# zongh5a/MDF-Net

Measured on AMD Instinct MI355X. Metric: views/sec at DTU 1600x1200x5-view x4-scale, higher is better.
Workload: dtype f32; 1 GPU; DTU eval 1600x1184 (1600x1200 cropped as load/dtueval.py:34), 5 views, 3 cost-volume stages + x2 refine = 4 output scales, hypotheses (48,24,8), batch 1 per rank, seeded random weights (pth/dtu_29.pth is not available offline); parallelism=views sharded over 1 rank(s), no collective

## Files before the change

### mdf-net_amd/csrc/conv3d.hip

```cpp
#include <cstdlib>
#include "common.h"

namespace {

typedef float f32x4 __attribute__((ext_vector_type(4)));

enum ConvMode { kS1 = 0, kS2 = 1, kTr = 2 };

struct ConvParams {
  const float* x;
  const float* wpack;
  const float* alpha;
  const float* beta;
  const float* res;
  float* y;
  int B, Di, Hi, Wi, Do, Ho, Wo;
  int relu;
  long long m_total;
  unsigned nblk;
  int stat_mode;
  const float* stat_y;
  const float* stat_aux;
  double* stat_out;
  int stat_slices;
// ... 708 lines not shown
  const int KPL = (Cin >= 16) ? 4 : (Cin == 8 ? 2 : 1), CK = 4 * KPL, NCH = Cin / CK, KW = KHW + RW - 1;
  int r = i;
  const int s = r % KPL; r /= KPL;
  const int n = r % 16; r /= 16;
  const int qq = r % 4; r /= 4;
  const int ch = r % NCH; r /= NCH;
  const int kwp = r % KW, kdh = r / KW;
  const int phase = n / Cout, cout = n % Cout, cin = ch * CK + KPL * qq + s;
  const int kw = kwp - phase;
  return (phase < RW && cin < Cin_mem && kw >= 0 && kw < KHW) ? src.at(cout, cin, kdh * KHW + kw) : 0.f;
}

__device__ __forceinline__ int pack_wino_total(int Cin, int Cout, int nkd) { return nkd * (Cin / 16) * 16 * ((Cout + 15) / 16) * 64 * 4; }
__device__ __forceinline__ float pack_wino_elem(const WSrc& src, int i, int Cin, int Cout, int nkd) {
  const int NCH = Cin / 16, NT = (Cout + 15) / 16;
  const float G[4][3] = {{1.f, 0.f, 0.f}, {.5f, .5f, .5f}, {.5f, -.5f, .5f}, {0.f, 0.f, 1.f}};
  int r = i;
  const int s = r % 4; r /= 4;
  const int m = r % 16; r /= 16;
  const int qq = r % 4; r /= 4;
  const int nt = r % NT; r /= NT;
  const int ab = r % 16; r /= 16;
  const int ch = r % NCH; r /= NCH;
  const int kd = r;
  const int a = ab >> 2, b = ab & 3;
  const int cout = nt * 16 + m, cin = ch * 16 + 4 * qq + s;
  float v = 0.f;
  if (cout < Cout) {
    for (int y = 0; y < 3; ++y)
      for (int x = 0; x < 3; ++x) v += G[a][y] * G[b][x] * src.at(cout, cin, kd * 9 + y * 3 + x);
  }
  return v;
}

__device__ __forceinline__ float pack_wd_elem(const WSrc& src, int i, int Cin) {
  const int KPL = (Cin >= 16) ? 4 : 2, CK = 4 * KPL, NCH = Cin / CK;
  const float G[4][3] = {{1.f, 0.f, 0.f}, {.5f, .5f, .5f}, {.5f, -.5f, .5f}, {0.f, 0.f, 1.f}};
  int r = i;
  const int s = r % KPL; r /= KPL;
  const int m = r % 16; r /= 16;
  const int qq = r % 4; r /= 4;
  const int ab = r % 16; r /= 16;
  const int ch = r % NCH; r /= NCH;
  const int j = r;
  const int a = ab >> 2, b = ab & 3;
  const int cout = m & 7, kd = j - (m >> 3), cin = ch * CK + KPL * qq + s;
  float v = 0.f;
  if (kd >= 0 && kd < 3) {
    for (int y = 0; y < 3; ++y)
      for (int x = 0; x < 3; ++x) v += G[a][y] * G[b][x] * src.at(cout, cin, kd * 9 + y * 3 + x);
  }
  return v;
}

__device__ __forceinline__ int pack_tr_total(int Cin, int Cout) {
  const int KPL = (Cin >= 16) ? 4 : 2, CK = 4 * KPL, NCH = Cin / CK, NT = (2 * Cout + 15) / 16;
  return 18 * NCH * NT * 64 * KPL;
}
__device__ __forceinline__ float pack_tr_elem(const WSrc& src, int i, int Cin, int Cout) {
  const int KPL = (Cin >= 16) ? 4 : 2, CK = 4 * KPL, NCH = Cin / CK, NT = (2 * Cout + 15) / 16;
  int r = i;
  const int s = r % KPL; r /= KPL;
  const int n = r % 16; r /= 16;
  const int qq = r % 4; r /= 4;
  const int nt = r % NT; r /= NT;
  const int ch = r % NCH; r /= NCH;
  const int tap = r;
  const int kd = tap / 6, kh = (tap / 2) % 3, ow = tap & 1;
  const int row = nt * 16 + n, cin = ch * CK + KPL * qq + s;
  if (row >= 2 * Cout) return 0.f;
  const int pw = row / Cout, cout = row % Cout;
  const int kw = (pw == 0) ? (ow == 0 ? 1 : -1) : (ow == 0 ? 2 : 0);
  return kw >= 0 ? src.at(cout, cin, (kd * 3 + kh) * 3 + kw) : 0.f;
}

__host__ __device__ inline int rw_of(int Cout) { return Cout == 8 ? 2 : (Cout == 4 ? 4 : 0); }
__host__ __device__ inline bool wino_built(int Cin, int Cout) {
  return ((Cout == 16 || Cout == 32) && (Cin == 16 || Cin == 32)) || (Cin == 16 && Cout == 8);
}
__host__ __device__ inline bool wino2d_built(int Cin, int Cout) {
  return (Cin == 16 && Cout == 16) || (Cin == 32 && Cout == 32) || (Cin == 64 && Cout == 64) || (Cin == 16 && Cout == 32) || (Cin == 32 && Cout == 64);
}
__host__ __device__ inline bool wd_built(int Cin, int Cout) { return Cout == 8 && (Cin == 8 || Cin == 16); }
__host__ __device__ inline bool k5w_built(int Cin, int Cout) { return (Cin == 16 && Cout == 32) || (Cin == 8 && Cout == 16); }
__host__ __device__ inline int padded_cin(int c) { return c <= 4 ? 4 : c; }

struct PackJob {
  const float* src;
  float* dst;
  int mode, transposed, is3d, Cin_mem, Cout, ntaps, a0, a1;
  int blk0, nblk;
};
__host__ __device__ inline void pack_segments(int is3d, int transposed, int Cin_mem, int Cout, int ntaps, long long* plain, long long* rw, long long* wino,
                                              long long* wd) {
  const int Cin = padded_cin(Cin_mem);
  const int KPL = (Cin >= 16) ? 4 : (Cin == 8 ? 2 : 1), NCH = Cin / (4 * KPL);
  *rw = 0; *wino = 0; *wd = 0;
  if (transposed) {
    const int K2 = (Cin >= 16) ? 4 : 2;
    *plain = 18ll * (Cin / (4 * K2)) * ((2 * Cout + 15) / 16) * 64 * K2;
    return;
  }
  *plain = (long long)ntaps * NCH * ((Cout + 15) / 16) * 64 * KPL;
  const bool k3 = is3d ? (ntaps == 27) : (ntaps == 9);
  if (k3 && rw_of(Cout)) *rw = (long long)(is3d ? 9 : 3) * (3 + rw_of(Cout) - 1) * NCH * 64 * KPL;
  if (k3 && (is3d ? wino_built(Cin_mem, Cout) : wino2d_built(Cin_mem, Cout))) *wino = (long long)(is3d ? 3 : 1) * (Cin / 16) * 16 * ((Cout + 15) / 16) * 64 * 4;
  if (k3 && is3d && wd_built(Cin_mem, Cout)) *wd = 4ll * NCH * 16 * 64 * KPL;
  if (!is3d && ntaps == 25 && k5w_built(Cin_mem, Cout)) *wino = (long long)(4 * Cin / 16) * 16 * ((Cout + 15) / 16) * 64 * 4;
}
__device__ __forceinline__ void pack_job_elem(const PackJob& j, long long i) {
  const int Cin = padded_cin(j.Cin_mem);
  WSrc src{j.src, j.transposed ? kSrcSwap : j.mode, j.Cout, j.Cin_mem, j.ntaps, j.a0, j.a1};
  long long plain, rw, wino, wd;
  pack_segments(j.is3d, j.transposed, j.Cin_mem, j.Cout, j.ntaps, &plain, &rw, &wino, &wd);
  if (i >= plain + rw + wino + wd) return;
  float v;
  if (j.transposed) v = pack_tr_elem(src, (int)i, Cin, j.Cout);
  else if (i < plain) v = pack_plain_elem(src, (int)i, Cin, j.Cin_mem, j.Cout);
  else if (i < plain + rw) v = pack_rw_elem(src, (int)(i - plain), Cin, j.Cin_mem, j.Cout, 3, rw_of(j.Cout));
  else if (i < plain + rw + wino) {
    if (!j.is3d && j.ntaps == 25) {
      const WSrc ph{j.src, kSrcK5S2Phases, j.Cout, 4 * j.Cin_mem, 9, j.Cin_mem, 0};
      v = (j.mode == kSrcDirect) ? pack_wino_elem(ph, (int)(i - plain - rw), 4 * Cin, j.Cout, 1) : 0.f;
    } else {
      v = pack_wino_elem(src, (int)(i - plain - rw), Cin, j.Cout, j.is3d ? 3 : 1);
    }
  }
  else v = pack_wd_elem(src, (int)(i - plain - rw - wino), Cin);
  j.dst[i] = v;
}

__global__ void pack_weights_kernel(PackJob j) {
  long long plain, rw, wino, wd;
  pack_segments(j.is3d, j.transposed, j.Cin_mem, j.Cout, j.ntaps, &plain, &rw, &wino, &wd);
  const long long total = plain + rw + wino + wd;
  for (long long i = (long long)blockIdx.x * blockDim.x + threadIdx.x; i < total; i += (long long)gridDim.x * blockDim.x) pack_job_elem(j, i);
}

constexpr int kPackPerBlock = 1024;
__global__ void pack_batch_kernel(const PackJob* __restrict__ jobs, const int* __restrict__ block_job) {
  const PackJob j = jobs[block_job[blockIdx.x]];
  const long long base = (long long)(blockIdx.x - j.blk0) * kPackPerBlock;
#pragma unroll
  for (int k = 0; k < kPackPerBlock / 256; ++k) pack_job_elem(j, base + k * 256 + threadIdx.x);
}

template <int CIN, int COUT, int MODE, int MT, int ST>
__global__ __launch_bounds__(1024) void conv3d_wlds_kernel(const ConvParams p) {
  constexpr int KPL = (CIN >= 16) ? 4 : 2, CK = 4 * KPL, NCH = CIN / CK, NT = (COUT + 15) / 16;
  constexpr int TAPF = NCH * NT * 64 * KPL;
  static_assert(MODE == kS1 || MODE == kS2, "stride-1 / stride-2 layers");
  extern __shared__ float wsm[];
  {
    const float4* src = reinterpret_cast<const float4*>(p.wpack);
    float4* dst = reinterpret_cast<float4*>(wsm);
    for (int i = threadIdx.x; i < 27 * TAPF / 4; i += 1024) dst[i] = src[i];
  }
  __shared__ double st_tab[ST ? 128 : 1];
  __shared__ float st_aux[ST ? 256 : 1];
  if constexpr (ST != 0) {
    if (threadIdx.x < 128) st_tab[threadIdx.x] = 0.0;
    if (p.stat_mode == 2 && threadIdx.x < 256) {
      const int c = threadIdx.x & 63;
      st_aux[threadIdx.x] = (c < COUT) ? p.stat_aux[(threadIdx.x >> 6) * COUT + c] : 0.f;
    }
  }
  __syncthreads();
// ... 471 lines not shown
```

### mdf-net_amd/csrc/conv_lds.hip

```cpp
#include <cstdlib>
#include <mutex>
#include <type_traits>
#include "common.h"

#include "conv_lds_common.h"

namespace {

constexpr int kSchedSlots = 128;
__device__ unsigned g_sched[2 * kSchedSlots];
#ifdef MDF_STAMPS
__device__ unsigned long long g_stamps[8];
#define STAMP() __builtin_readcyclecounter()
#endif

template <typename C, int KD, int KHW, int SHW, int COUT, int MTL, int ST = 0>
__device__ __forceinline__ void step(const float* const (&planes)[KD], __amdgpu_buffer_rsrc_t wres, int wvoff, const LdsConvParams& p,
                                     size_t row_vox, int w0, int q, int n16, const float (&wr)[C::WN][C::NT][C::KPL],
                                     const float (&al)[C::NT][4], const float (&be)[C::NT][4], const float (&wfirst)[2][C::NT][C::KPL]) {
  constexpr int NT = C::NT;
  extern __shared__ __attribute__((aligned(16))) float lds_base_[];
  const float* epi_tab = lds_base_ + C::EPI_OFF;
  static_assert(ST == 0 || COUT % 4 == 0, "epilogue sums need Cout % 4 == 0");
  f32x4 acc[MTL][NT];
// ... 784 lines not shown

static int sched_slot_of(void* stream) {
  std::lock_guard<std::mutex> lock(g_slot_mu);
  int free_slot = -1;
  for (int i = 0; i < kSchedSlots; ++i) {
    if (g_slot_used[i] && g_slot_stream[i] == stream) return i;
    if (!g_slot_used[i] && free_slot < 0) free_slot = i;
  }
  if (free_slot >= 0) { g_slot_used[free_slot] = true; g_slot_stream[free_slot] = stream; }
  return free_slot;
}

extern "C" int mdf_release_stream(void* stream) {
  std::lock_guard<std::mutex> lock(g_slot_mu);
  for (int i = 0; i < kSchedSlots; ++i)
    if (g_slot_used[i] && g_slot_stream[i] == stream) { g_slot_used[i] = false; g_slot_stream[i] = nullptr; return MDF_OK; }
  return MDF_OK;
}

#define LDS_CASE_RW(ci, cim, co, kd, k, s, mt, rw)                                               \
  if (!stat && use_rw && Cin == ci && Cin_mem == cim && Cout == co && KD == kd && KHW == k && stride == s && !res_up) { \
    p.wpack = wpack + (size_t)kd * k * k * ci * 16;                                              \
    return launch_lds<ci, cim, co, kd, k, s, mt, rw>(p, (hipStream_t)stream);                    \
  }
#define LDS_CASE_RW_T(ci, cim, co, kd, k, s, mt, rw)                                             \
  if (use_rw && Cin == ci && Cin_mem == cim && Cout == co && KD == kd && KHW == k && stride == s && !res_up) { \
    p.wpack = wpack + (size_t)kd * k * k * ci * 16;                                              \
    return !stat ? launch_lds<ci, cim, co, kd, k, s, mt, rw>(p, (hipStream_t)stream) : (stat->mode == 1 ? launch_lds<ci, cim, co, kd, k, s, mt, rw, 0, 1>(p, (hipStream_t)stream) : launch_lds<ci, cim, co, kd, k, s, mt, rw, 0, 2>(p, (hipStream_t)stream)); \
  }

#define LDS_CASE_WG(ci, co)                                                                      \
  if (use_wg && KD == 3 && KHW == 3 && stride == 1 && Cin == ci && Cin_mem == ci && Cout == co && !res_up) { \
    p.wpack = wpack + (size_t)27 * ci * (((co + 15) / 16) * 16) + (co == 8 ? (size_t)36 * ci * 16 : 0); \
    return !stat ? launch_lds<ci, ci, co, 3, 3, 1, 1, 2, 1>(p, (hipStream_t)stream) : (stat->mode == 1 ? launch_lds<ci, ci, co, 3, 3, 1, 1, 2, 1, 1>(p, (hipStream_t)stream) : launch_lds<ci, ci, co, 3, 3, 1, 1, 2, 1, 2>(p, (hipStream_t)stream)); \
  }
#define LDS_CASE_WG2(ci, co)                                                                     \
  if (use_wg && KD == 1 && KHW == 3 && stride == 1 && Cin == ci && Cin_mem == ci && Cout == co && !res_up && (!shuffle2 || (ci == 16 && co == 32) || (ci == 32 && co == 64))) { \
    p.wpack = wpack + (size_t)9 * ci * (((co + 15) / 16) * 16);                                  \
    return !stat ? launch_lds<ci, ci, co, 1, 3, 1, 1, 2, 1>(p, (hipStream_t)stream) : (stat->mode == 1 ? launch_lds<ci, ci, co, 1, 3, 1, 1, 2, 1, 1>(p, (hipStream_t)stream) : launch_lds<ci, ci, co, 1, 3, 1, 1, 2, 1, 2>(p, (hipStream_t)stream)); \
  }

#define LDS_CASE_WD(ci)                                                                          \
  if (use_wd && KD == 3 && KHW == 3 && stride == 1 && Cin == ci && Cin_mem == ci && Cout == 8 && !res_up && D >= 2) { \
    p.wpack = wpack + (size_t)27 * ci * 16 + (size_t)36 * ci * 16 + (ci == 16 ? (size_t)3 * 16 * 64 * 4 : 0); \
    if (ci == 16 && wd_stream && !stat) return launch_lds<ci, ci, 8, 3, 3, 1, 1, 2, 3>(p, (hipStream_t)stream); \
    return !stat ? launch_lds<ci, ci, 8, 3, 3, 1, 1, 2, 2>(p, (hipStream_t)stream) : (stat->mode == 1 ? launch_lds<ci, ci, 8, 3, 3, 1, 1, 2, 2, 1>(p, (hipStream_t)stream) : launch_lds<ci, ci, 8, 3, 3, 1, 1, 2, 2, 2>(p, (hipStream_t)stream)); \
  }

int mdf_wino3d_dispatch(const float* x, const float* wpack_wino, const float* alpha, const float* beta, const float* res, float res_scale,
                        float* y, int B, int D, int H, int W, int Cin, int Cout, int relu, void* stream);
int mdf_wino2d_dispatch(const float* x, const float* wpack_wino, const float* alpha, const float* beta, const float* res, float res_scale,
                        float* y, int B, int H, int W, int Cin, int Cout, int relu, void* stream);
int mdf_wino2d_s2d_dispatch(const float* x, const float* wpack_k5w, const float* alpha, const float* beta, float* y, int B, int Ho, int Wo,
                            int Cin_mem, int Cout, int relu, void* stream);

int mdf_conv_lds_dispatch(const float* x, const float* wpack, const float* alpha, const float* beta, const float* res,
                          float res_scale, const float* res_up, float* y, int B, int D, int H, int W, int Cin, int Cin_mem, int Cout, int KD,
                          int KHW, int stride, int relu, void* stream, int planar_in, int shuffle2, const mdf::ConvStat* stat) {
  static const int wd_mask = [] { const char* e = getenv("MDF_CONV_WD"); return e ? atoi(e) : 3; }();
  const bool wd_stream = [] { const char* e = getenv("MDF_CONV_WD_STREAM"); return e ? atoi(e) != 0 : true; }();
  static const bool use_wg = [] { const char* e = getenv("MDF_CONV_WINOGRAD"); return e ? atoi(e) != 0 : true; }();
  static const bool use_rw = [] { const char* e = getenv("MDF_CONV_RW"); return e ? atoi(e) != 0 : true; }();
  LdsConvParams p{};
  p.x = x; p.wpack = wpack; p.alpha = alpha; p.beta = beta; p.res = res; p.res_scale = res_scale; p.res_up = res_up; p.y = y;
  p.B = B; p.D = D; p.H = H; p.W = W; p.relu = relu; p.planar_in = planar_in; p.shuffle2 = shuffle2;
  if (stat) {
    if (Cout % 4 != 0 || shuffle2 || res_up) return mdf::fail(MDF_EUNSUPPORTED, "epilogue sums: Cout %% 4 == 0, no pixel-shuffle / upsample-add");
    p.stat_mode = stat->mode; p.stat_y = stat->y; p.stat_aux = stat->aux; p.stat_out = stat->out; p.stat_slices = stat->nslices;
    p.stat_groups = (KD == 1 && stat->group_imgs > 0) ? B / stat->group_imgs : 1;
  }
  p.sched_slot = sched_slot_of(stream);
  if (p.sched_slot < 0) return mdf::fail(MDF_EUNSUPPORTED, "conv kernels support up to %d distinct HIP streams per process", kSchedSlots);
  {
    const char* e = getenv("MDF_CONV_PREFETCH_EARLY");
    p.prefetch_early = e ? atoi(e) : 0;
  }
  const int pad = (KHW - 1) / 2;
  p.Ho = (H + 2 * pad - KHW) / stride + 1;
  p.Wo = (W + 2 * pad - KHW) / stride + 1;
  {
    const bool k5w = [] { const char* e = getenv("MDF_CONV_K5_WINOGRAD"); return e ? atoi(e) != 0 : true; }();
    if (use_wg && k5w && KD == 1 && KHW == 5 && stride == 2 && !stat && !res_up && !shuffle2 && !planar_in && H % 2 == 0 && W % 2 == 0) {
      const bool use_w2 = [] { const char* e = getenv("MDF_CONV_WINO2D"); return e ? atoi(e) != 0 : true; }();
      if (use_w2 && !res && Cin == Cin_mem && ((Cin == 16 && Cout == 32) || (Cin == 8 && Cout == 16))) {
        const size_t plain = (size_t)25 * 64 * (Cin == 16 ? 2 * 4 : 1 * 2);
        const int rc = mdf_wino2d_s2d_dispatch(x, wpack + plain, alpha, beta, y, B, p.Ho, p.Wo, Cin, Cout, relu, stream);
        if (rc != MDF_EUNSUPPORTED) return rc;
      }
      if (Cin == 16 && Cin_mem == 16 && Cout == 32) {
        p.s2d = 1; p.wpack = wpack + (size_t)25 * 1 * 2 * 64 * 4;
        return launch_lds<64, 64, 32, 1, 3, 1, 1, 2, 1>(p, (hipStream_t)stream);
      }
    }
  }
  if (shuffle2 && Cout == 64 && !use_wg) return mdf::fail(MDF_EUNSUPPORTED, "pixel-shuffle store for Cout = 64 is built into the Winograd form only (MDF_CONV_WINOGRAD=0 is set)");
  { const bool use_wd = use_wg && (wd_mask & 1); LDS_CASE_WD(8) }
  { const bool use_wd = use_wg && (wd_mask & 2); LDS_CASE_WD(16) }
  {
    const bool use_w3 = [] { const char* e = getenv("MDF_CONV_WINO3D"); return e ? atoi(e) != 0 : true; }();
    if (use_wg && use_w3 && !stat && KD == 3 && KHW == 3 && stride == 1 && Cin == Cin_mem && !res_up && !shuffle2 && Cout % 16 == 0) {
      const int rc = mdf_wino3d_dispatch(x, wpack + (size_t)27 * Cin * Cout, alpha, beta, res, res_scale, y, B, D, H, W, Cin, Cout, relu, stream);
      if (rc != MDF_EUNSUPPORTED) return rc;
    }
  }
  {
    const bool use_w2 = [] { const char* e = getenv("MDF_CONV_WINO2D"); return e ? atoi(e) != 0 : true; }();
    if (use_wg && use_w2 && !stat && KD == 1 && KHW == 3 && stride == 1 && Cin == Cin_mem && !res_up && !shuffle2 && !planar_in && D == 1) {
      const int rc = mdf_wino2d_dispatch(x, wpack + (size_t)9 * Cin * (((Cout + 15) / 16) * 16), alpha, beta, res, res_scale, y, B, H, W, Cin, Cout, relu, stream);
      if (rc != MDF_EUNSUPPORTED) return rc;
    }
  }
  LDS_CASE_WG(16, 16) LDS_CASE_WG(32, 16) LDS_CASE_WG(32, 32) LDS_CASE_WG(16, 8) LDS_CASE_WG(16, 32)
  LDS_CASE_WG2(16, 16) LDS_CASE_WG2(32, 32) LDS_CASE_WG2(64, 64) LDS_CASE_WG2(16, 32) LDS_CASE_WG2(32, 64)
  LDS_CASE_RW_T(16, 16, 8, 3, 3, 1, 2, 2) LDS_CASE_RW_T(8, 8, 8, 3, 3, 1, 2, 2)
  LDS_CASE_RW(16, 16, 4, 1, 3, 1, 1, 4) LDS_CASE_RW(8, 8, 4, 1, 3, 1, 1, 4)
  LDS_CASE_RW_T(8, 8, 8, 1, 3, 1, 2, 2) LDS_CASE_RW_T(4, 3, 8, 1, 3, 1, 2, 2) LDS_CASE_RW(4, 1, 8, 1, 3, 1, 2, 2)
  LDS_CASE(32, 32, 16, 3, 3, 1, 2) LDS_CASE(16, 16, 16, 3, 3, 1, 4) LDS_CASE(16, 16, 8, 3, 3, 1, 4) LDS_CASE(8, 8, 8, 3, 3, 1, 4)
  LDS_CASE(32, 32, 32, 3, 3, 1, 2)
  LDS_CASE(16, 16, 32, 3, 3, 1, 2) LDS_CASE(8, 8, 16, 3, 3, 1, 4)
  LDS_CASE(4, 3, 8, 1, 3, 1, 4) LDS_CASE(8, 8, 8, 1, 3, 1, 4) LDS_CASE(16, 16, 16, 1, 3, 1, 4) LDS_CASE(32, 32, 32, 1, 3, 1, 2)
  LDS_CASE(64, 64, 64, 1, 3, 1, 1)
  LDS_CASE_T(8, 8, 16, 1, 5, 2, 2) LDS_CASE_T(16, 16, 32, 1, 5, 2, 2) LDS_CASE_T(32, 32, 64, 1, 5, 2, 1)
  LDS_CASE(16, 16, 32, 1, 1, 1, 4)
  LDS_CASE(16, 16, 64, 1, 1, 1, 4) LDS_CASE(32, 32, 64, 1, 1, 1, 2) LDS_CASE(64, 64, 16, 1, 1, 1, 1) LDS_CASE(64, 64, 32, 1, 1, 1, 1)
  LDS_CASE(64, 64, 64, 1, 1, 1, 1)
  LDS_CASE(32, 32, 32, 1, 1, 1, 2) LDS_CASE(32, 32, 16, 1, 1, 1, 2) LDS_CASE(16, 16, 16, 1, 1, 1, 4)
  LDS_CASE(4, 1, 8, 1, 3, 1, 4) LDS_CASE(8, 8, 32, 1, 3, 1, 4) LDS_CASE(8, 8, 1, 1, 3, 1, 4)
  LDS_CASE(32, 32, 8, 1, 3, 1, 2)
  LDS_CASE(16, 16, 32, 1, 3, 1, 2) LDS_CASE(32, 32, 64, 1, 3, 1, 1)
  LDS_CASE(16, 16, 4, 1, 3, 1, 4) LDS_CASE(8, 8, 4, 1, 3, 1, 4)
  return MDF_EUNSUPPORTED;
}
```

### mdf-net_amd/csrc/wino2d.hip

```cpp
#include <cstdlib>
#include <type_traits>
#include "common.h"
#include "conv_lds_common.h"
#define W3_PINNED_TILES_32
#include "wino3d_acc.h"

namespace {

template <int I, int N, typename F>
__device__ __forceinline__ void static_for(F&& f) {
  if constexpr (I < N) {
    f(std::integral_constant<int, I>{});
    static_for<I + 1, N>(f);
  }
}

struct Wino2dParams {
  const float* x;
  const float* wpack;
  const float* alpha;
  const float* beta;
  const float* res;
  float* y;
  float res_scale;
  int B, H, W, relu;
  int tiles_h, tiles_w, n_tiles;
};

template <int CIN, int COUT>
struct W2 {
  static_assert(CIN % 16 == 0 && COUT % 16 == 0 && COUT <= 64, "2-D Winograd form: Cin, Cout multiples of 16, Cout <= 64");
  static constexpr int NCH = CIN / 16, NT = COUT / 16, NG = CIN / 4;
  static constexpr int WN = (CIN >= 64) ? 2 : 1, NTW = NT / WN, WM = 4 / WN;
  static_assert(NT % WN == 0 && NTW >= 1 && NTW <= 2, "cout tiles per wave");
  static constexpr int TH = 2 * WM, TWO = 32;
  static constexpr int PH = TH + 2, PW = TWO + 2;
  static constexpr int NPP = PH * PW;
  static constexpr int S = round_s(NPP, 4, 2);
  static constexpr int PLANE = CIN * S;
  static constexpr int RING = 3;
  static constexpr int NPOS = NG * NPP;
  static constexpr int NFILL = (NPOS + 255) / 256;
  static constexpr int EPI_OFF = RING * PLANE;
  static constexpr int FRAG = 64 * 4;
  static constexpr int NSTEP = NCH * 16;
  static constexpr bool WL = ((size_t)(RING * PLANE + 128 + NSTEP * NT * FRAG) * sizeof(float) <= 160 * 1024);
  static constexpr int W_OFF = EPI_OFF + 128;
  static constexpr size_t LDS_BYTES = (size_t)(RING * PLANE + 128 + (WL ? NSTEP * NT * FRAG : 0)) * sizeof(float);
  static_assert(S > NPP, "a pad vector per group takes the fill's surplus lanes");
};

#ifndef MDF_W2_DIAG
#define MDF_W2_DIAG 0
#endif
#ifndef MDF_W2_HOLD_REL
#define MDF_W2_HOLD_REL 0
#endif
#ifndef MDF_W2_NA
#define MDF_W2_NA 4
#endif
#ifndef MDF_W2_WRITE_AB
#define MDF_W2_WRITE_AB 2
#endif

template <int CIN, int COUT, int NA, int WRITE_AB, bool S2D>
__global__ __launch_bounds__(256, 1) void wino2d_kernel(const Wino2dParams p) {
  typedef W2<CIN, COUT> C;
  constexpr int NCH = C::NCH, NT = C::NT, S = C::S, PW = C::PW, NPP = C::NPP, NFILL = C::NFILL, NSTEP = C::NSTEP;
  constexpr int AH = NA - 1;
  static_assert(NSTEP % NA == 0, "the fragment ring must close over a tile");
  extern __shared__ __attribute__((aligned(16))) float lds[];

  const int tid = threadIdx.x, lane = tid & 63;
  const int wave = __builtin_amdgcn_readfirstlane(tid >> 6);
  const int q = lane >> 4, n16 = lane & 15;
  const __amdgpu_buffer_rsrc_t wres = make_rsrc(p.wpack, (unsigned)(NSTEP * NT * 64 * 4 * 4));
  const int wvoff = lane * 16;
  const int wm = wave / C::WN, wn = wave % C::WN;
  constexpr int NTW = C::NTW;
  const int lane_lds = (q * S + wm * 2 * PW + n16 * 2) * 4;

  if (tid < 128) {
    const int c = tid & 63;
    lds[C::EPI_OFF + tid] = (tid < 64) ? ((c < COUT && p.alpha) ? p.alpha[c] : 1.f) : ((c < COUT && p.beta) ? p.beta[c] : 0.f);
  }
  if constexpr (C::WL) {
    constexpr int NV = NSTEP * NT * 64;
    for (int v = tid; v < NV; v += 256)
      *reinterpret_cast<float4*>(lds + C::W_OFF + v * 4) = *reinterpret_cast<const float4*>(p.wpack + (size_t)v * 4);
  }

  constexpr bool HOLD_REL = (NFILL <= 11) || (NTW == 1) || MDF_W2_HOLD_REL;
  constexpr int CM = S2D ? CIN / 4 : CIN;
  [[maybe_unused]] constexpr int GPP = CM / 4;
  auto rel_of = [&](int row, int col, int g) -> int {
    if constexpr (S2D) {
      const int par = g / GPP, c4 = g - par * GPP;
      return (((2 * row + (par >> 1)) * (2 * p.W) + 2 * col + (par & 1)) * CM + c4 * 4) * 4;
    } else {
      return ((row * p.W + col) * CIN + g * 4) * 4;
    }
  };
  int f_lds[NFILL], f_rc[NFILL], f_rel[HOLD_REL ? NFILL : 1];
#pragma unroll
  for (int k = 0; k < NFILL; ++k) {
    const int idx = tid + k * 256;
    const int glo = idx & 3, r = idx >> 2;
    const int v = r % NPP, g = (r / NPP) * 4 + glo;
    const bool live = idx < C::NPOS;
    const int row = live ? v / PW : 0x40, col = v % PW;
    f_lds[k] = live ? (g * S + v) * 4 : NPP * 4;
    f_rc[k] = (row << 16) | (col << 8) | g;
    if constexpr (HOLD_REL) f_rel[k] = live ? rel_of(row, col, g) : (int)0x80000000u;
  }

  const unsigned lb = mdf::xcd_remap(blockIdx.x, gridDim.x);
  const int t_begin = __builtin_amdgcn_readfirstlane((int)((unsigned long long)lb * (unsigned)p.n_tiles / gridDim.x));
  const int t_end = __builtin_amdgcn_readfirstlane((int)((unsigned long long)(lb + 1) * (unsigned)p.n_tiles / gridDim.x));
  if (t_begin >= t_end) return;

  float4 pf[NFILL];
  struct TileAt { int b, th, tw; };
  auto tile_at = [&](int t) -> TileAt {
    const int tw = t % p.tiles_w, rest = t / p.tiles_w;
    return TileAt{__builtin_amdgcn_readfirstlane(rest / p.tiles_h), __builtin_amdgcn_readfirstlane(rest % p.tiles_h), __builtin_amdgcn_readfirstlane(tw)};
  };
  auto tile_advance = [&](TileAt& c) {
    if (++c.tw == p.tiles_w) {
      c.tw = 0;
      if (++c.th == p.tiles_h) { c.th = 0; ++c.b; }
    }
  };
  auto issue_tile = [&](const TileAt& at, bool valid) {
    const int b = valid ? at.b : 0, h0 = (valid ? at.th : 0) * C::TH, w0 = (valid ? at.tw : 0) * C::TWO;
    const long long org = S2D ? ((long long)b * (2 * p.H) + 2 * (h0 - 1)) * (2 * p.W) + 2 * (w0 - 1)
                              : ((long long)b * p.H + (h0 - 1)) * p.W + (w0 - 1);
    const float* pz = p.x + org * CM;
    const unsigned long long pa = (unsigned long long)pz;
    const unsigned lo = (unsigned)__builtin_amdgcn_readfirstlane((int)(unsigned)pa), hi = (unsigned)__builtin_amdgcn_readfirstlane((int)(unsigned)(pa >> 32));
    const unsigned nrec = (!valid || (MDF_W2_DIAG & 1)) ? 0u : 0x7fffffffu;
    const __amdgpu_buffer_rsrc_t xr = make_rsrc((const void*)(((unsigned long long)hi << 32) | lo), nrec);
    const int r_lo = 1 - h0, r_hi = p.H + 1 - h0, c_lo = 1 - w0, c_hi = p.W + 1 - w0;
    if constexpr (HOLD_REL) {
      if (r_lo <= 0 && r_hi >= C::PH && c_lo <= 0 && c_hi >= C::PW) {
#pragma unroll
        for (int k = 0; k < NFILL; ++k) {
          const u32x4_t v = __builtin_amdgcn_raw_buffer_load_b128(xr, f_rel[k], 0, 0);
          pf[k] = make_float4(__uint_as_float(v.x), __uint_as_float(v.y), __uint_as_float(v.z), __uint_as_float(v.w));
        }
        return;
      }
    }
#pragma unroll
    for (int k = 0; k < NFILL; ++k) {
      const int row = f_rc[k] >> 16, col = (f_rc[k] >> 8) & 0xff;
      const bool ok = row >= r_lo && row < r_hi && col >= c_lo && col < c_hi;
      int rel;
      if constexpr (HOLD_REL) rel = f_rel[k];
      else rel = rel_of(row, col, f_rc[k] & 0xff);
      const u32x4_t v = __builtin_amdgcn_raw_buffer_load_b128(xr, ok ? rel : (int)0x80000000u, 0, 0);
      pf[k] = make_float4(__uint_as_float(v.x), __uint_as_float(v.y), __uint_as_float(v.z), __uint_as_float(v.w));
    }
  };
  auto write_tile = [&](int slot) {
#pragma unroll
    for (int k = 0; k < NFILL; ++k) *reinterpret_cast<float4*>(lds + slot * C::PLANE + f_lds[k]) = pf[k];
  };

  f32x2_t V[16][2], Dn[16][2];
  auto read_elem = [&](int slot, int ch, int e) {
    const int i = e >> 2, j = e & 3;
    float t[4];
    lds_frag<4>(lds + slot * C::PLANE + lane_lds + ((ch * 4) * S + i * PW + j) * 4, t);
    Dn[e][0] = (f32x2_t){t[0], t[1]};
    Dn[e][1] = (f32x2_t){t[2], t[3]};
  };
  auto transform = [&]() {
#pragma unroll
    for (int j = 0; j < 4; ++j)
#pragma unroll
      for (int c = 0; c < 2; ++c) {
        const f32x2_t d0 = Dn[j][c], d1 = Dn[4 + j][c], d2 = Dn[8 + j][c], d3 = Dn[12 + j][c];
        Dn[j][c] = d0 - d2; Dn[4 + j][c] = d1 + d2; Dn[8 + j][c] = d2 - d1; Dn[12 + j][c] = d1 - d3;
      }
#pragma unroll
    for (int a = 0; a < 4; ++a)
#pragma unroll
      for (int c = 0; c < 2; ++c) {
        const f32x2_t e0 = Dn[a * 4][c], e1 = Dn[a * 4 + 1][c], e2 = Dn[a * 4 + 2][c], e3 = Dn[a * 4 + 3][c];
        V[a * 4][c] = e0 - e2; V[a * 4 + 1][c] = e1 + e2; V[a * 4 + 2][c] = e2 - e1; V[a * 4 + 3][c] = e1 - e3;
      }
#pragma unroll
    for (int e = 0; e < 16; ++e)
#pragma unroll
      for (int c = 0; c < 2; ++c) asm volatile("" : "+v"(V[e][c]));
  };

  float af[NA][NTW][4];
  auto load_a = [&](int i, int buf) {
#pragma unroll
    for (int ntl = 0; ntl < NTW; ++ntl) {
      if constexpr (C::WL) lds_frag<4>(lds + C::W_OFF + (i * NT + wn * NTW + ntl) * C::FRAG + lane * 4, af[buf][ntl]);
      else buf_load_to<4>(wres, wvoff, (i * NT + wn * NTW + ntl) * (64 * 4 * 4), af[buf][ntl]);
    }
  };

  auto epilogue = [&](const TileAt& at) {
    const int b = at.b, h0 = at.th * C::TH, w0 = at.tw * C::TWO;
    if (h0 + 2 * wm >= p.H) return;
    const float* epi_tab = lds + C::EPI_OFF;
    asm volatile("s_nop 15\n\ts_nop 15" ::: "memory");
    static_for<0, NTW>([&](auto ntc) {
      constexpr int nt = decltype(ntc)::value;
      const int c0 = (wn * NTW + nt) * 16 + 4 * q;
      float yv[2][2][4];
      static_for<0, 2>([&](auto k2c) {
        constexpr int k2 = decltype(k2c)::value;
        float m[16][2];
        static_for<0, 16>([&](auto abc) { AccTile<nt * 16 + decltype(abc)::value>::template read2<k2>(m[decltype(abc)::value]); });
        f32x2_t srow[2][4];
#pragma unroll
        for (int bb = 0; bb < 4; ++bb) {
          const f32x2_t m0 = {m[bb][0], m[bb][1]}, m1 = {m[4 + bb][0], m[4 + bb][1]};
          const f32x2_t m2 = {m[8 + bb][0], m[8 + bb][1]}, m3 = {m[12 + bb][0], m[12 + bb][1]};
          srow[0][bb] = m0 + m1 + m2;
          srow[1][bb] = m1 - m2 - m3;
        }
#pragma unroll
        for (int pr = 0; pr < 2; ++pr) {
          const f32x2_t y0 = srow[pr][0] + srow[pr][1] + srow[pr][2];
          const f32x2_t y1 = srow[pr][1] - srow[pr][2] - srow[pr][3];
          yv[pr][0][2 * k2] = y0[0]; yv[pr][0][2 * k2 + 1] = y0[1];
          yv[pr][1][2 * k2] = y1[0]; yv[pr][1][2 * k2 + 1] = y1[1];
        }
      });
      float al_l[4], be_l[4];
#pragma unroll
      for (int k = 0; k < 4; ++k) { al_l[k] = epi_tab[c0 + k]; be_l[k] = epi_tab[64 + c0 + k]; }
#pragma unroll
      for (int pr = 0; pr < 2; ++pr) {
        const int h = h0 + 2 * wm + pr;
        if (h >= p.H) continue;
        const size_t row_vox = ((size_t)b * p.H + h) * p.W;
#pragma unroll
        for (int rr = 0; rr < 2; ++rr) {
          const int ow = w0 + 2 * n16 + rr;
          if (ow >= p.W) continue;
          float ov[4];
#pragma unroll
          for (int k = 0; k < 4; ++k) {
            ov[k] = yv[pr][rr][k] * al_l[k] + be_l[k];
            if (p.relu) ov[k] = fmaxf(ov[k], 0.f);
          }
          const size_t oi = (row_vox + ow) * COUT + c0;
          if (p.res) {
            const float4 rv = *reinterpret_cast<const float4*>(p.res + oi);
            ov[0] = rv.x + ov[0] * p.res_scale; ov[1] = rv.y + ov[1] * p.res_scale;
            ov[2] = rv.z + ov[2] * p.res_scale; ov[3] = rv.w + ov[3] * p.res_scale;
          }
          if (!(MDF_W2_DIAG & 2) || ov[0] == 1234.5f) *reinterpret_cast<float4*>(p.y + oi) = make_float4(ov[0], ov[1], ov[2], ov[3]);
        }
      }
    });
  };

  auto step = [&](auto rc, const TileAt& at, const TileAt& at_next2, bool valid_next2, bool has_next) {
    constexpr int R = decltype(rc)::value;
    constexpr int SLOT_N = (R + 1) % 3;
    static_for<0, NSTEP>([&](auto ic) {
      constexpr int i = decltype(ic)::value;
      constexpr int ch = i / 16, ab = i % 16;
      constexpr bool last_chunk = (ch == NCH - 1);
      if (!(MDF_W2_DIAG & 16)) load_a((i + AH) % NSTEP, (i + AH) % NA);
      if constexpr (ch == 0 && ab == WRITE_AB) {
        if (has_next) {
          write_tile(SLOT_N);
          __syncthreads();
        }
      }
      if constexpr (ab > WRITE_AB && ab <= WRITE_AB + 8 && !(MDF_W2_DIAG & 32)) {
        constexpr int e0 = 2 * (ab - WRITE_AB - 1);
        if constexpr (!last_chunk) { read_elem(R, ch + 1, e0); read_elem(R, ch + 1, e0 + 1); }
        else { read_elem(SLOT_N, 0, e0); read_elem(SLOT_N, 0, e0 + 1); }
      }
      __builtin_amdgcn_sched_barrier(0);
      static_for<0, NTW>([&](auto ntc) {
        constexpr int nt = decltype(ntc)::value;
        constexpr int T = nt * 16 + ab;
        if constexpr (ch == 0) AccTile<T>::mfma_fresh(af[i % NA][nt][0], V[ab][0][0]);
        else AccTile<T>::mfma(af[i % NA][nt][0], V[ab][0][0]);
        AccTile<T>::mfma(af[i % NA][nt][1], V[ab][0][1]);
        AccTile<T>::mfma(af[i % NA][nt][2], V[ab][1][0]);
        AccTile<T>::mfma(af[i % NA][nt][3], V[ab][1][1]);
      });
      __builtin_amdgcn_sched_barrier(0);
      if constexpr (ab == 15 && !last_chunk) { if (!(MDF_W2_DIAG & 8)) transform(); }
    });
    issue_tile(at_next2, valid_next2);
    if (!(MDF_W2_DIAG & 8)) transform();
    if (!(MDF_W2_DIAG & 4)) epilogue(at);
  };

  int t = t_begin;
  const int t_last = t_end - 1;
  TileAt at = tile_at(t), at2 = at;
  issue_tile(at, true);
  write_tile(0);
  __syncthreads();
  tile_advance(at2);
  issue_tile(at2, t < t_last);
  tile_advance(at2);
#pragma unroll
  for (int e = 0; e < 16; ++e) read_elem(0, 0, e);
  transform();
#pragma unroll
  for (int i = 0; i < AH; ++i) load_a(i, i % NA);

#define W2_STEP(RR)                                                                        \
  {                                                                                        \
    const bool has_next = t < t_last;                                                      \
    step(std::integral_constant<int, RR>{}, at, at2, t + 2 <= t_last, has_next);           \
    if (!has_next) break;                                                                  \
    ++t; tile_advance(at); tile_advance(at2);                                              \
  }
  for (;;) {
    W2_STEP(0)
    W2_STEP(1)
    W2_STEP(2)
  }
#undef W2_STEP
}

template <int CIN, int COUT, bool S2D = false>
int launch_wino2d(Wino2dParams& p, hipStream_t st) {
  typedef W2<CIN, COUT> C;
  constexpr int NA = MDF_W2_NA, WRITE_AB = MDF_W2_WRITE_AB;
  p.tiles_h = (p.H + C::TH - 1) / C::TH;
  p.tiles_w = (p.W + C::TWO - 1) / C::TWO;
  const long long tiles = (long long)p.B * p.tiles_h * p.tiles_w;
  if (tiles >= (1ll << 31)) return MDF_EUNSUPPORTED;
  p.n_tiles = (int)tiles;
  auto kern = &wino2d_kernel<CIN, COUT, NA, WRITE_AB, S2D>;
  static bool attr_done_dev[64] = {};
  int dev_id = 0;
  (void)hipGetDevice(&dev_id);
  bool& attr_done = attr_done_dev[(dev_id >= 0 && dev_id < 64) ? dev_id : 0];
  if (!attr_done || dev_id >= 64) {
    hipError_t e = hipFuncSetAttribute(reinterpret_cast<const void*>(kern), hipFuncAttributeMaxDynamicSharedMemorySize, (int)C::LDS_BYTES);
    if (e != hipSuccess) return mdf::fail(MDF_EHIP, "hipFuncSetAttribute(dynamic LDS %zu): %s", (size_t)C::LDS_BYTES, hipGetErrorString(e));
    attr_done = true;
  }
  long long grid = 256;
  if (const char* g = getenv("MDF_WINO2D_GRID")) { if (atoi(g) > 0) grid = atoi(g); }
  if (grid > tiles / 2) grid = tiles / 2;
  if (grid < 1) grid = 1;
  hipLaunchKernelGGL(kern, dim3((unsigned)grid), dim3(256), C::LDS_BYTES, st, p);
  return mdf::check_launch("wino2d_kernel");
}

}

int mdf_wino2d_dispatch(const float* x, const float* wpack_wino, const float* alpha, const float* beta, const float* res, float res_scale,
                        float* y, int B, int H, int W, int Cin, int Cout, int relu, void* stream) {
  Wino2dParams p{};
  p.x = x; p.wpack = wpack_wino; p.alpha = alpha; p.beta = beta; p.res = res; p.res_scale = res_scale; p.y = y;
  p.B = B; p.H = H; p.W = W; p.relu = relu;
  if ((long long)B * H * W * Cin * 4 >= (1ll << 31)) return MDF_EUNSUPPORTED;
  if (Cin == 16 && Cout == 16 && getenv("MDF_WINO2D_16")) return launch_wino2d<16, 16>(p, (hipStream_t)stream);
  if (Cin == 32 && Cout == 32) return launch_wino2d<32, 32>(p, (hipStream_t)stream);
  if (Cin == 64 && Cout == 64) return launch_wino2d<64, 64>(p, (hipStream_t)stream);
  return MDF_EUNSUPPORTED;
}

int mdf_wino2d_s2d_dispatch(const float* x, const float* wpack_k5w, const float* alpha, const float* beta, float* y, int B, int Ho, int Wo,
                            int Cin_mem, int Cout, int relu, void* stream) {
  Wino2dParams p{};
  p.x = x; p.wpack = wpack_k5w; p.alpha = alpha; p.beta = beta; p.res = nullptr; p.res_scale = 0.f; p.y = y;
  p.B = B; p.H = Ho; p.W = Wo; p.relu = relu;
  if ((long long)B * Ho * Wo * 4 * Cin_mem * 4 >= (1ll << 31)) return MDF_EUNSUPPORTED;
  if (Cin_mem == 16 && Cout == 32) return launch_wino2d<64, 32, true>(p, (hipStream_t)stream);
  if (Cin_mem == 8 && Cout == 16) return launch_wino2d<32, 16, true>(p, (hipStream_t)stream);
  return MDF_EUNSUPPORTED;
}
```

Before: 297.2 views/s.

## Extend space-to-depth Winograd to 32->64 k5s2 conv with parity-zero step skipping

Routes the 5x5 stride-2 conv with 32 input and 64 output channels through the 2-D Winograd space-to-depth kernel. Its 128 parity channels are processed in two passes so LDS fits. Also adds compile-time skipping of Winograd transform elements and MFMA steps that are identically zero for odd-parity sub-channels, applied to the 16->32 path as well. The intent is to cut wasted MFMA and transform work and move a larger layer onto the faster path. In exchange it adds complex pipeline bookkeeping (padding steps, per-pass tile issue) that could hurt scheduling or register pressure.

```diff
diff --git a/mdf-net_amd/csrc/conv3d.hip b/mdf-net_amd/csrc/conv3d.hip
--- a/mdf-net_amd/csrc/conv3d.hip
+++ b/mdf-net_amd/csrc/conv3d.hip
@@ -814,7 +814,7 @@
   return (Cin == 16 && Cout == 16) || (Cin == 32 && Cout == 32) || (Cin == 64 && Cout == 64) || (Cin == 16 && Cout == 32) || (Cin == 32 && Cout == 64);
 }
 __host__ __device__ inline bool wd_built(int Cin, int Cout) { return Cout == 8 && (Cin == 8 || Cin == 16); }
-__host__ __device__ inline bool k5w_built(int Cin, int Cout) { return (Cin == 16 && Cout == 32) || (Cin == 8 && Cout == 16); }
+__host__ __device__ inline bool k5w_built(int Cin, int Cout) { return (Cin == 32 && Cout == 64) || (Cin == 16 && Cout == 32) || (Cin == 8 && Cout == 16); }
 __host__ __device__ inline int padded_cin(int c) { return c <= 4 ? 4 : c; }
 
 struct PackJob {
diff --git a/mdf-net_amd/csrc/conv_lds.hip b/mdf-net_amd/csrc/conv_lds.hip
--- a/mdf-net_amd/csrc/conv_lds.hip
+++ b/mdf-net_amd/csrc/conv_lds.hip
@@ -890,8 +890,9 @@
     const bool k5w = [] { const char* e = getenv("MDF_CONV_K5_WINOGRAD"); return e ? atoi(e) != 0 : true; }();
     if (use_wg && k5w && KD == 1 && KHW == 5 && stride == 2 && !stat && !res_up && !shuffle2 && !planar_in && H % 2 == 0 && W % 2 == 0) {
       const bool use_w2 = [] { const char* e = getenv("MDF_CONV_WINO2D"); return e ? atoi(e) != 0 : true; }();
-      if (use_w2 && !res && Cin == Cin_mem && ((Cin == 16 && Cout == 32) || (Cin == 8 && Cout == 16))) {
-        const size_t plain = (size_t)25 * 64 * (Cin == 16 ? 2 * 4 : 1 * 2);
+      const bool k5w64 = [] { const char* e = getenv("MDF_CONV_K5_WINOGRAD_64"); return e ? atoi(e) != 0 : true; }();
+      if (use_w2 && !res && Cin == Cin_mem && ((Cin == 32 && Cout == 64 && k5w64) || (Cin == 16 && Cout == 32) || (Cin == 8 && Cout == 16))) {
+        const size_t plain = (size_t)25 * 64 * (Cin == 32 ? 2 * 4 * 4 : (Cin == 16 ? 2 * 4 : 1 * 2));
         const int rc = mdf_wino2d_s2d_dispatch(x, wpack + plain, alpha, beta, y, B, p.Ho, p.Wo, Cin, Cout, relu, stream);
         if (rc != MDF_EUNSUPPORTED) return rc;
       }
diff --git a/mdf-net_amd/csrc/wino2d.hip b/mdf-net_amd/csrc/wino2d.hip
--- a/mdf-net_amd/csrc/wino2d.hip
+++ b/mdf-net_amd/csrc/wino2d.hip
@@ -29,25 +29,67 @@
 
 template <int CIN, int COUT>
 struct W2 {
-  static_assert(CIN % 16 == 0 && COUT % 16 == 0 && COUT <= 64, "2-D Winograd form: Cin, Cout multiples of 16, Cout <= 64");
-  static constexpr int NCH = CIN / 16, NT = COUT / 16, NG = CIN / 4;
-  static constexpr int WN = (CIN >= 64) ? 2 : 1, NTW = NT / WN, WM = 4 / WN;
+  static_assert(CIN % 16 == 0 && COUT % 16 == 0 && COUT <= 64 && CIN <= 128, "2-D Winograd form: Cin, Cout multiples of 16, Cout <= 64");
+  static constexpr int PASSES = (CIN > 64) ? 2 : 1, CP = CIN / PASSES;
+  static constexpr int NCH = CP / 16, NT = COUT / 16, NG = CP / 4;
+  static constexpr int WN = (CP >= 64) ? 2 : 1, NTW = NT / WN, WM = 4 / WN;
   static_assert(NT % WN == 0 && NTW >= 1 && NTW <= 2, "cout tiles per wave");
   static constexpr int TH = 2 * WM, TWO = 32;
   static constexpr int PH = TH + 2, PW = TWO + 2;
   static constexpr int NPP = PH * PW;
   static constexpr int S = round_s(NPP, 4, 2);
-  static constexpr int PLANE = CIN * S;
+  static constexpr int PLANE = CP * S;
   static constexpr int RING = 3;
   static constexpr int NPOS = NG * NPP;
   static constexpr int NFILL = (NPOS + 255) / 256;
   static constexpr int EPI_OFF = RING * PLANE;
   static constexpr int FRAG = 64 * 4;
   static constexpr int NSTEP = NCH * 16;
-  static constexpr bool WL = ((size_t)(RING * PLANE + 128 + NSTEP * NT * FRAG) * sizeof(float) <= 160 * 1024);
+  static constexpr bool WL = ((size_t)(RING * PLANE + 128 + PASSES * NSTEP * NT * FRAG) * sizeof(float) <= 160 * 1024);
   static constexpr int W_OFF = EPI_OFF + 128;
-  static constexpr size_t LDS_BYTES = (size_t)(RING * PLANE + 128 + (WL ? NSTEP * NT * FRAG : 0)) * sizeof(float);
+  static constexpr size_t LDS_BYTES = (size_t)(RING * PLANE + 128 + (WL ? PASSES * NSTEP * NT * FRAG : 0)) * sizeof(float);
   static_assert(S > NPP, "a pad vector per group takes the fill's surplus lanes");
+};
+
+template <int CIN, bool S2D, bool SKIP, int PAD = 0>
+struct W2Live {
+  static constexpr int CM = CIN / 4, NSTEP = CIN;
+  static constexpr bool all_odd(int ch, int bit) {
+    for (int c = ch * 16; c < ch * 16 + 16; ++c)
+      if (!(((c / CM) >> bit) & 1)) return false;
+    return true;
+  }
+  static constexpr bool py1(int ch) { return S2D && SKIP && all_odd(ch, 1); }
+  static constexpr bool px1(int ch) { return S2D && SKIP && all_odd(ch, 0); }
+  static constexpr bool zero(int ch, int ab) { return (py1(ch) && (ab >> 2) == 3) || (px1(ch) && (ab & 3) == 3); }
+  static constexpr bool kept(int ch, int ab) {
+    if (!zero(ch, ab)) return false;
+    int n = 0;
+    for (int i = 0; i < ch * 16 + ab; ++i) n += zero(i / 16, i % 16) ? 1 : 0;
+    return n < PAD;
+  }
+  static constexpr bool dead(int ch, int ab) { return zero(ch, ab) && !kept(ch, ab); }
+  static constexpr bool kept_ok() {
+    for (int i = 0; i < NSTEP; ++i)
+      if (kept(i / 16, i % 16) && (i % 16 == 0 || zero(i / 16, i % 16 - 1))) return false;
+    return true;
+  }
+  static constexpr bool need(int ch, int e) { return !(py1(ch) && (e >> 2) == 3) && !(px1(ch) && (e & 3) == 3); }
+  static constexpr int count(int upto = NSTEP) {
+    int n = 0;
+    for (int i = 0; i < upto; ++i) n += dead(i / 16, i % 16) ? 0 : 1;
+    return n;
+  }
+  static constexpr int nth(int j) {
+    for (int i = 0; i < NSTEP; ++i)
+      if (!dead(i / 16, i % 16) && j-- == 0) return i;
+    return -1;
+  }
+  static constexpr bool chunk0_live() {
+    for (int ab = 0; ab < 16; ++ab)
+      if (dead(0, ab)) return false;
+    return true;
+  }
 };
 
 #ifndef MDF_W2_DIAG
@@ -63,18 +105,23 @@
 #define MDF_W2_WRITE_AB 2
 #endif
 
-template <int CIN, int COUT, int NA, int WRITE_AB, bool S2D>
+template <int CIN, int COUT, int NA, int WRITE_AB, bool S2D, bool SKIP = true, int PAD = 0>
 __global__ __launch_bounds__(256, 1) void wino2d_kernel(const Wino2dParams p) {
   typedef W2<CIN, COUT> C;
-  constexpr int NCH = C::NCH, NT = C::NT, S = C::S, PW = C::PW, NPP = C::NPP, NFILL = C::NFILL, NSTEP = C::NSTEP;
+  typedef W2Live<CIN, S2D, SKIP, PAD> LV;
+  constexpr int NCH = C::NCH, NT = C::NT, S = C::S, PW = C::PW, NPP = C::NPP, NFILL = C::NFILL, NSTEP = C::NSTEP, PASSES = C::PASSES;
   constexpr int AH = NA - 1;
-  static_assert(NSTEP % NA == 0, "the fragment ring must close over a tile");
+  constexpr int NL = LV::count();
+  static_assert(PASSES * NSTEP == LV::NSTEP && (PASSES == 1 || S2D), "passes: the parity form only");
+  static_assert(NA >= 2 && NL % NA == 0, "the fragment ring must close over a tile");
+  static_assert(LV::chunk0_live(), "every accumulator tile's first step is in chunk 0 of pass 0 (mfma_fresh)");
+  static_assert(LV::kept_ok(), "a kept zero step has a computed V[ab - 1]");
   extern __shared__ __attribute__((aligned(16))) float lds[];
 
   const int tid = threadIdx.x, lane = tid & 63;
   const int wave = __builtin_amdgcn_readfirstlane(tid >> 6);
   const int q = lane >> 4, n16 = lane & 15;
-  const __amdgpu_buffer_rsrc_t wres = make_rsrc(p.wpack, (unsigned)(NSTEP * NT * 64 * 4 * 4));
+  const __amdgpu_buffer_rsrc_t wres = make_rsrc(p.wpack, (unsigned)(PASSES * NSTEP * NT * 64 * 4 * 4));
   const int wvoff = lane * 16;
   const int wm = wave / C::WN, wn = wave % C::WN;
   constexpr int NTW = C::NTW;
@@ -85,7 +132,7 @@
     lds[C::EPI_OFF + tid] = (tid < 64) ? ((c < COUT && p.alpha) ? p.alpha[c] : 1.f) : ((c < COUT && p.beta) ? p.beta[c] : 0.f);
   }
   if constexpr (C::WL) {
-    constexpr int NV = NSTEP * NT * 64;
+    constexpr int NV = PASSES * NSTEP * NT * 64;
     for (int v = tid; v < NV; v += 256)
       *reinterpret_cast<float4*>(lds + C::W_OFF + v * 4) = *reinterpret_cast<const float4*>(p.wpack + (size_t)v * 4);
   }
@@ -93,9 +140,10 @@
   constexpr bool HOLD_REL = (NFILL <= 11) || (NTW == 1) || MDF_W2_HOLD_REL;
   constexpr int CM = S2D ? CIN / 4 : CIN;
   [[maybe_unused]] constexpr int GPP = CM / 4;
-  auto rel_of = [&](int row, int col, int g) -> int {
+  static_assert(HOLD_REL ? PASSES == 1 : true, "held offsets are those of pass 0");
+  auto rel_of = [&](int row, int col, int g, int pass) -> int {
     if constexpr (S2D) {
-      const int par = g / GPP, c4 = g - par * GPP;
+      const int gl = pass * C::NG + g, par = gl / GPP, c4 = gl - par * GPP;
       return (((2 * row + (par >> 1)) * (2 * p.W) + 2 * col + (par & 1)) * CM + c4 * 4) * 4;
     } else {
       return ((row * p.W + col) * CIN + g * 4) * 4;
@@ -111,7 +159,7 @@
     const int row = live ? v / PW : 0x40, col = v % PW;
     f_lds[k] = live ? (g * S + v) * 4 : NPP * 4;
     f_rc[k] = (row << 16) | (col << 8) | g;
-    if constexpr (HOLD_REL) f_rel[k] = live ? rel_of(row, col, g) : (int)0x80000000u;
+    if constexpr (HOLD_REL) f_rel[k] = live ? rel_of(row, col, g, 0) : (int)0x80000000u;
   }
 
   const unsigned lb = mdf::xcd_remap(blockIdx.x, gridDim.x);
@@ -131,7 +179,7 @@
       if (++c.th == p.tiles_h) { c.th = 0; ++c.b; }
     }
   };
-  auto issue_tile = [&](const TileAt& at, bool valid) {
+  auto issue_tile = [&](const TileAt& at, int pass, bool valid) {
     const int b = valid ? at.b : 0, h0 = (valid ? at.th : 0) * C::TH, w0 = (valid ? at.tw : 0) * C::TWO;
     const long long org = S2D ? ((long long)b * (2 * p.H) + 2 * (h0 - 1)) * (2 * p.W) + 2 * (w0 - 1)
                               : ((long long)b * p.H + (h0 - 1)) * p.W + (w0 - 1);
@@ -157,7 +205,7 @@
       const bool ok = row >= r_lo && row < r_hi && col >= c_lo && col < c_hi;
       int rel;
       if constexpr (HOLD_REL) rel = f_rel[k];
-      else rel = rel_of(row, col, f_rc[k] & 0xff);
+      else rel = rel_of(row, col, f_rc[k] & 0xff, pass);
       const u32x4_t v = __builtin_amdgcn_raw_buffer_load_b128(xr, ok ? rel : (int)0x80000000u, 0, 0);
       pf[k] = make_float4(__uint_as_float(v.x), __uint_as_float(v.y), __uint_as_float(v.z), __uint_as_float(v.w));
     }
@@ -175,25 +223,31 @@
     Dn[e][0] = (f32x2_t){t[0], t[1]};
     Dn[e][1] = (f32x2_t){t[2], t[3]};
   };
-  auto transform = [&]() {
-#pragma unroll
-    for (int j = 0; j < 4; ++j)
+  auto transform = [&](auto lcc) {
+    constexpr int LC = decltype(lcc)::value;
+    constexpr bool PY = LV::py1(LC), PX = LV::px1(LC);
+#pragma unroll
+    for (int j = 0; j < (PX ? 3 : 4); ++j)
 #pragma unroll
       for (int c = 0; c < 2; ++c) {
-        const f32x2_t d0 = Dn[j][c], d1 = Dn[4 + j][c], d2 = Dn[8 + j][c], d3 = Dn[12 + j][c];
-        Dn[j][c] = d0 - d2; Dn[4 + j][c] = d1 + d2; Dn[8 + j][c] = d2 - d1; Dn[12 + j][c] = d1 - d3;
-      }
-#pragma unroll
-    for (int a = 0; a < 4; ++a)
+        const f32x2_t d0 = Dn[j][c], d1 = Dn[4 + j][c], d2 = Dn[8 + j][c];
+        Dn[j][c] = d0 - d2; Dn[4 + j][c] = d1 + d2; Dn[8 + j][c] = d2 - d1;
+        if constexpr (!PY) { const f32x2_t d3 = Dn[12 + j][c]; Dn[12 + j][c] = d1 - d3; }
+      }
+#pragma unroll
+    for (int a = 0; a < (PY ? 3 : 4); ++a)
 #pragma unroll
       for (int c = 0; c < 2; ++c) {
-        const f32x2_t e0 = Dn[a * 4][c], e1 = Dn[a * 4 + 1][c], e2 = Dn[a * 4 + 2][c], e3 = Dn[a * 4 + 3][c];
-        V[a * 4][c] = e0 - e2; V[a * 4 + 1][c] = e1 + e2; V[a * 4 + 2][c] = e2 - e1; V[a * 4 + 3][c] = e1 - e3;
-      }
-#pragma unroll
-    for (int e = 0; e < 16; ++e)
+        const f32x2_t e0 = Dn[a * 4][c], e1 = Dn[a * 4 + 1][c], e2 = Dn[a * 4 + 2][c];
+        V[a * 4][c] = e0 - e2; V[a * 4 + 1][c] = e1 + e2; V[a * 4 + 2][c] = e2 - e1;
+        if constexpr (!PX) { const f32x2_t e3 = Dn[a * 4 + 3][c]; V[a * 4 + 3][c] = e1 - e3; }
+      }
+#pragma unroll
+    for (int e = 0; e < 16; ++e) {
+      if ((PY && (e >> 2) == 3) || (PX && (e & 3) == 3)) continue;
 #pragma unroll
       for (int c = 0; c < 2; ++c) asm volatile("" : "+v"(V[e][c]));
+    }
   };
 
   float af[NA][NTW][4];
@@ -264,14 +318,21 @@
     });
   };
 
-  auto step = [&](auto rc, const TileAt& at, const TileAt& at_next2, bool valid_next2, bool has_next) {
-    constexpr int R = decltype(rc)::value;
+  auto step = [&](auto rc, auto pc, const TileAt& at, const TileAt& at_n, bool valid_n, bool has_next) {
+    constexpr int R = decltype(rc)::value, P = decltype(pc)::value;
     constexpr int SLOT_N = (R + 1) % 3;
+    constexpr int LC_NEXT = (P + 1 < PASSES) ? (P + 1) * NCH : 0;
     static_for<0, NSTEP>([&](auto ic) {
       constexpr int i = decltype(ic)::value;
       constexpr int ch = i / 16, ab = i % 16;
+      constexpr int lc = P * NCH + ch, li = P * NSTEP + i;
       constexpr bool last_chunk = (ch == NCH - 1);
-      if (!(MDF_W2_DIAG & 16)) load_a((i + AH) % NSTEP, (i + AH) % NA);
+      constexpr bool live = !LV::dead(lc, ab);
+      [[maybe_unused]] constexpr int j = LV::count(li);
+      if constexpr (live) {
+        constexpr int ahead = LV::nth((j + AH) % NL);
+        if (!(MDF_W2_DIAG & 16)) load_a(ahead, (j + AH) % NA);
+      }
       if constexpr (ch == 0 && ab == WRITE_AB) {
         if (has_next) {
           write_tile(SLOT_N);
@@ -280,67 +341,96 @@
       }
       if constexpr (ab > WRITE_AB && ab <= WRITE_AB + 8 && !(MDF_W2_DIAG & 32)) {
         constexpr int e0 = 2 * (ab - WRITE_AB - 1);
-        if constexpr (!last_chunk) { read_elem(R, ch + 1, e0); read_elem(R, ch + 1, e0 + 1); }
-        else { read_elem(SLOT_N, 0, e0); read_elem(SLOT_N, 0, e0 + 1); }
+        constexpr int lcn = last_chunk ? LC_NEXT : lc + 1;
+        static_for<0, 2>([&](auto kc) {
+          constexpr int e = e0 + decltype(kc)::value;
+          if constexpr (LV::need(lcn, e)) {
+            if constexpr (!last_chunk) read_elem(R, ch + 1, e);
+            else read_elem(SLOT_N, 0, e);
+          }
+        });
       }
       __builtin_amdgcn_sched_barrier(0);
-      static_for<0, NTW>([&](auto ntc) {
-        constexpr int nt = decltype(ntc)::value;
-        constexpr int T = nt * 16 + ab;
-        if constexpr (ch == 0) AccTile<T>::mfma_fresh(af[i % NA][nt][0], V[ab][0][0]);
-        else AccTile<T>::mfma(af[i % NA][nt][0], V[ab][0][0]);
-        AccTile<T>::mfma(af[i % NA][nt][1], V[ab][0][1]);
-        AccTile<T>::mfma(af[i % NA][nt][2], V[ab][1][0]);
-        AccTile<T>::mfma(af[i % NA][nt][3], V[ab][1][1]);
-      });
+      if constexpr (live) {
+        static_for<0, NTW>([&](auto ntc) {
+          constexpr int nt = decltype(ntc)::value;
+          constexpr int T = nt * 16 + ab;
+          constexpr int vb = LV::kept(lc, ab) ? ab - 1 : ab;
+          if constexpr (lc == 0) AccTile<T>::mfma_fresh(af[j % NA][nt][0], V[vb][0][0]);
+          else AccTile<T>::mfma(af[j % NA][nt][0], V[vb][0][0]);
+          AccTile<T>::mfma(af[j % NA][nt][1], V[vb][0][1]);
+          AccTile<T>::mfma(af[j % NA][nt][2], V[vb][1][0]);
+          AccTile<T>::mfma(af[j % NA][nt][3], V[vb][1][1]);
+        });
+      }
       __builtin_amdgcn_sched_barrier(0);
-      if constexpr (ab == 15 && !last_chunk) { if (!(MDF_W2_DIAG & 8)) transform(); }
+      if constexpr (ab == 15 && !last_chunk) { if (!(MDF_W2_DIAG & 8)) transform(std::integral_constant<int, lc + 1>{}); }
     });
-    issue_tile(at_next2, valid_next2);
-    if (!(MDF_W2_DIAG & 8)) transform();
-    if (!(MDF_W2_DIAG & 4)) epilogue(at);
+    issue_tile(at_n, P, valid_n);
+    if (!(MDF_W2_DIAG & 8)) transform(std::integral_constant<int, LC_NEXT>{});
+    if constexpr (P == PASSES - 1) { if (!(MDF_W2_DIAG & 4)) epilogue(at); }
   };
 
   int t = t_begin;
   const int t_last = t_end - 1;
   TileAt at = tile_at(t), at2 = at;
-  issue_tile(at, true);
+  issue_tile(at, 0, true);
   write_tile(0);
   __syncthreads();
   tile_advance(at2);
-  issue_tile(at2, t < t_last);
-  tile_advance(at2);
+  if constexpr (PASSES == 1) {
+    issue_tile(at2, 0, t < t_last);
+    tile_advance(at2);
+  } else {
+    issue_tile(at, 1, true);
+  }
 #pragma unroll
   for (int e = 0; e < 16; ++e) read_elem(0, 0, e);
-  transform();
-#pragma unroll
-  for (int i = 0; i < AH; ++i) load_a(i, i % NA);
-
-#define W2_STEP(RR)                                                                        \
-  {                                                                                        \
-    const bool has_next = t < t_last;                                                      \
-    step(std::integral_constant<int, RR>{}, at, at2, t + 2 <= t_last, has_next);           \
-    if (!has_next) break;                                                                  \
-    ++t; tile_advance(at); tile_advance(at2);                                              \
-  }
-  for (;;) {
-    W2_STEP(0)
-    W2_STEP(1)
-    W2_STEP(2)
+  transform(std::integral_constant<int, 0>{});
+  static_for<0, AH>([&](auto ic) {
+    constexpr int first = LV::nth(decltype(ic)::value);
+    load_a(first, decltype(ic)::value % NA);
+  });
+
+#define W2_STEP(RR, PP)                                                                                                          \
+  {                                                                                                                              \
+    const bool more = t < t_last;                                                                                                \
+    if constexpr (PASSES == 1) step(std::integral_constant<int, RR>{}, std::integral_constant<int, 0>{}, at, at2, t + 2 <= t_last, more); \
+    else step(std::integral_constant<int, RR>{}, std::integral_constant<int, PP>{}, at, at2, more, (PP) == 0 || more);           \
+    if constexpr ((PP) == PASSES - 1) {                                                                                          \
+      if (!more) break;                                                                                                          \
+      ++t; tile_advance(at); tile_advance(at2);                                                                                  \
+    }                                                                                                                            \
+  }
+  if constexpr (PASSES == 1) {
+    for (;;) {
+      W2_STEP(0, 0)
+      W2_STEP(1, 0)
+      W2_STEP(2, 0)
+    }
+  } else {
+    for (;;) {
+      W2_STEP(0, 0)
+      W2_STEP(1, 1)
+      W2_STEP(2, 0)
+      W2_STEP(0, 1)
+      W2_STEP(1, 0)
+      W2_STEP(2, 1)
+    }
   }
 #undef W2_STEP
 }
 
-template <int CIN, int COUT, bool S2D = false>
+template <int CIN, int COUT, bool S2D = false, bool SKIP = true, int NA = MDF_W2_NA, int PAD = 0>
 int launch_wino2d(Wino2dParams& p, hipStream_t st) {
   typedef W2<CIN, COUT> C;
-  constexpr int NA = MDF_W2_NA, WRITE_AB = MDF_W2_WRITE_AB;
+  constexpr int WRITE_AB = MDF_W2_WRITE_AB;
   p.tiles_h = (p.H + C::TH - 1) / C::TH;
   p.tiles_w = (p.W + C::TWO - 1) / C::TWO;
   const long long tiles = (long long)p.B * p.tiles_h * p.tiles_w;
   if (tiles >= (1ll << 31)) return MDF_EUNSUPPORTED;
   p.n_tiles = (int)tiles;
-  auto kern = &wino2d_kernel<CIN, COUT, NA, WRITE_AB, S2D>;
+  auto kern = &wino2d_kernel<CIN, COUT, NA, WRITE_AB, S2D, S2D && SKIP, PAD>;
   static bool attr_done_dev[64] = {};
   int dev_id = 0;
   (void)hipGetDevice(&dev_id);
@@ -378,7 +468,10 @@
   p.x = x; p.wpack = wpack_k5w; p.alpha = alpha; p.beta = beta; p.res = nullptr; p.res_scale = 0.f; p.y = y;
   p.B = B; p.H = Ho; p.W = Wo; p.relu = relu;
   if ((long long)B * Ho * Wo * 4 * Cin_mem * 4 >= (1ll << 31)) return MDF_EUNSUPPORTED;
-  if (Cin_mem == 16 && Cout == 32) return launch_wino2d<64, 32, true>(p, (hipStream_t)stream);
-  if (Cin_mem == 8 && Cout == 16) return launch_wino2d<32, 16, true>(p, (hipStream_t)stream);
+  const bool skip = [] { const char* e = getenv("MDF_WINO2D_SKIP"); return e ? atoi(e) != 0 : true; }();
+  hipStream_t st = (hipStream_t)stream;
+  if (Cin_mem == 32 && Cout == 64) return skip ? launch_wino2d<128, 64, true, true, 4, 2>(p, st) : launch_wino2d<128, 64, true, false>(p, st);
+  if (Cin_mem == 16 && Cout == 32) return skip ? launch_wino2d<64, 32, true, true, 7, 0>(p, st) : launch_wino2d<64, 32, true, false>(p, st);
+  if (Cin_mem == 8 && Cout == 16) return launch_wino2d<32, 16, true, false>(p, st);
   return MDF_EUNSUPPORTED;
 }
```

Measured after the change: 303.3 views/s (median of 6 runs). +2.1%, better.
